# kshedden/muscato

Measured on AMD Instinct MI355X. Metric: reads/sec (100 bp, multi-map) at 1/2/4/8 MI355X; confirm-kernel HBM GB/s vs peak, higher is better.
Workload: dtype u32

## Files before the change

include/muscato_hip.h:

```cpp
#ifndef MUSCATO_HIP_H
#define MUSCATO_HIP_H

#include <stdint.h>

#ifdef __cplusplus
extern "C" {
#endif

#define MUSC_ABI_VERSION 3
#define MUSC_MAX_WINDOWS 16

typedef struct musc_ctx musc_ctx;

typedef struct {
  uint32_t read_idx;
  uint32_t gene_idx;
  uint32_t pos;
  uint32_t nmiss;
} musc_hit;

typedef struct {
  int32_t n_windows;
  int32_t windows[MUSC_MAX_WINDOWS];
  int32_t window_width;
// ... 53 lines not shown
int musc_db_build_index_for(musc_ctx* ctx, const musc_params* params, int32_t max_read_len);

int musc_db_set_partition_bases(musc_ctx* ctx, uint64_t max_bases);
int musc_db_partitions(musc_ctx* ctx, uint32_t* first_target, uint32_t cap, uint32_t* n);

int musc_reads_load_ascii(musc_ctx* ctx, const char* seqs, const uint64_t* offsets,
                          uint64_t nreads, int on_device);
int musc_reads_load_packed(musc_ctx* ctx, const uint8_t* bases2bit, const uint8_t* nmask,
                           const uint64_t* read_offsets, uint64_t nreads);
int musc_reads_load_packed32(musc_ctx* ctx, const uint8_t* bases2bit, const uint8_t* nmask,
                             const uint32_t* lengths, uint32_t fixed_len, uint64_t nreads, int async);

int musc_reads_sort_unique(musc_ctx* ctx, const char* seqs, const uint64_t* offsets, uint64_t nreads,
                           int on_device, uint32_t** order, uint32_t** ustart, uint64_t* nunique);

typedef struct musc_fastq_prep {
  uint64_t n_records, n_short, n_reads, n_unique;
  uint32_t max_len, reserved;
  uint64_t *name_off, *seq_off;
  uint32_t *name_len, *seq_len;
  uint32_t *order, *ustart;
} musc_fastq_prep;
int  musc_reads_prep_fastq(musc_ctx* ctx, const char* text, uint64_t nbytes, int on_device,
                           int32_t min_read_len, int32_t max_read_len, musc_fastq_prep* out);
void musc_fastq_prep_free(musc_fastq_prep* p);

int musc_reads_names_order(musc_ctx* ctx, const char* text, uint64_t nbytes, int on_device, const uint64_t* name_off,
                           const uint32_t* name_len, uint64_t n, const uint32_t* order, const uint32_t* ustart, uint64_t nu,
                           uint32_t* ranked_out);
typedef struct musc_read_names {
// ... 103 lines not shown
```

muscato_amd/_lib.py:

```python
from __future__ import annotations

import ctypes
import os

HERE = os.path.dirname(os.path.abspath(__file__))
LIB_PATH = os.environ.get("MUSC_LIB_PATH") or os.path.join(HERE, "libmuscato_hip.so")

MUSC_MAX_WINDOWS = 16


class MuscHit(ctypes.Structure):
    _fields_ = [("read_idx", ctypes.c_uint32), ("gene_idx", ctypes.c_uint32),
                ("pos", ctypes.c_uint32), ("nmiss", ctypes.c_uint32)]


class MuscParams(ctypes.Structure):
    _fields_ = [
        ("n_windows", ctypes.c_int32),
        ("windows", ctypes.c_int32 * MUSC_MAX_WINDOWS),
        ("window_width", ctypes.c_int32),
        ("pmatch", ctypes.c_double),
        ("min_dinuc", ctypes.c_int32),
        ("max_read_length", ctypes.c_int32),
        ("max_matches", ctypes.c_int32),
# ... 55 lines not shown

class MuscTargetsPrepInfo(ctypes.Structure):
    _fields_ = [
        ("n_lines", ctypes.c_uint64), ("n_records", ctypes.c_uint64), ("n_targets", ctypes.c_uint64),
        ("n_dropped", ctypes.c_uint64), ("stop_line", ctypes.c_uint64), ("n_subx", ctypes.c_uint64),
        ("n_seq_bytes", ctypes.c_uint64), ("n_id_bytes", ctypes.c_uint64),
        ("ms", ctypes.c_float), ("reserved", ctypes.c_uint32),
    ]


SYMBOLS = [
    "musc_abi_version", "musc_init", "musc_destroy", "musc_last_error", "musc_reload_env",
    "musc_db_load_ascii", "musc_db_load_packed", "musc_db_build_index", "musc_db_build_index_for",
    "musc_db_set_partition_bases", "musc_db_partitions",
    "musc_reads_load_ascii", "musc_reads_load_packed", "musc_reads_load_packed32", "musc_reads_sort_unique",
    "musc_reads_prep_fastq", "musc_fastq_prep_free",
    "musc_reads_names_order", "musc_reads_prep_fastq_names", "musc_reads_names_text",
    "musc_match_device", "musc_hits_copy", "musc_hits_copy_packed", "musc_hits_copy_compact", "musc_hits_unpack", "musc_match", "musc_free_hits",
    "musc_get_stats", "musc_last_instance", "musc_instances", "musc_stream_plan", "musc_gather", "musc_gather_rccl", "musc_rccl_probe", "musc_overflow_probes", "musc_free_u32",
    "musc_results_set_gene_text", "musc_results_set_read_text", "musc_results_order", "musc_results_hits", "musc_results_text",
    "musc_results_last_ms", "musc_results_number_key",
    "musc_side_prepare", "musc_side_text", "musc_side_last_ms",
    "musc_maxmatches_apply", "musc_maxmatches_last_ms", "musc_maxmatches_last_detail",
    "musc_sz_decode", "musc_db_load_text",
    "musc_targets_prep", "musc_targets_prep_text", "musc_targets_prep_load", "musc_targets_prep_free", "musc_sz_frame",
]

SIDE_NONMATCH, SIDE_GENESTATS, SIDE_READSTATS = 0, 1, 2

_lib = None

# ... 25 lines not shown
    lib.musc_destroy.restype = None
    lib.musc_last_error.argtypes = [vp]
    lib.musc_last_error.restype = ctypes.c_char_p
    lib.musc_reload_env.argtypes = [vp]
    lib.musc_db_load_ascii.argtypes = [vp, vp, vp, ctypes.c_uint32, ctypes.c_int]
    lib.musc_db_load_packed.argtypes = [vp, vp, vp, vp, ctypes.c_uint32]
    lib.musc_db_build_index.argtypes = [vp, i32]
    lib.musc_db_build_index_for.argtypes = [vp, ctypes.POINTER(MuscParams), i32]
    lib.musc_db_set_partition_bases.argtypes = [vp, u64]
    lib.musc_db_partitions.argtypes = [vp, vp, ctypes.c_uint32, ctypes.POINTER(ctypes.c_uint32)]
    lib.musc_reads_load_ascii.argtypes = [vp, vp, vp, u64, ctypes.c_int]
    lib.musc_reads_load_packed.argtypes = [vp, vp, vp, vp, u64]
    lib.musc_reads_load_packed32.argtypes = [vp, vp, vp, vp, ctypes.c_uint32, u64, ctypes.c_int]
    lib.musc_reads_sort_unique.argtypes = [vp, vp, vp, u64, ctypes.c_int, ctypes.POINTER(vp), ctypes.POINTER(vp),
                                           ctypes.POINTER(u64)]
    lib.musc_reads_prep_fastq.argtypes = [vp, vp, u64, ctypes.c_int, i32, i32, ctypes.POINTER(MuscFastqPrep)]
    lib.musc_reads_prep_fastq.restype = ctypes.c_int
    lib.musc_fastq_prep_free.argtypes = [ctypes.POINTER(MuscFastqPrep)]
    lib.musc_fastq_prep_free.restype = None
    lib.musc_reads_names_order.argtypes = [vp, vp, u64, ctypes.c_int, vp, vp, u64, vp, vp, u64, vp]
    lib.musc_reads_prep_fastq_names.argtypes = [vp, vp, u64, ctypes.c_int, i32, i32, ctypes.POINTER(MuscFastqPrep), ctypes.POINTER(MuscReadNames)]
    lib.musc_reads_names_text.argtypes = [vp, ctypes.c_int, u64, u64, vp, u64, ctypes.c_int, ctypes.POINTER(u64)]
    for name in ("musc_reads_names_order", "musc_reads_prep_fastq_names", "musc_reads_names_text"):
        getattr(lib, name).restype = ctypes.c_int
    lib.musc_match_device.argtypes = [vp, ctypes.POINTER(MuscParams), ctypes.POINTER(u64)]
    lib.musc_hits_copy.argtypes = [vp, vp, u64, ctypes.c_int]
    lib.musc_hits_copy_packed.argtypes = [vp, vp, u64, ctypes.c_int, u64, ctypes.POINTER(i32)]
    lib.musc_hits_copy_compact.argtypes = [vp, vp, u64, vp, u64, ctypes.c_int, ctypes.POINTER(i32)]
    lib.musc_hits_unpack.argtypes = [vp, vp, u64, ctypes.c_int, ctypes.POINTER(i32), vp]
    lib.musc_match.argtypes = [vp, ctypes.POINTER(MuscParams), ctypes.POINTER(vp), ctypes.POINTER(u64)]
# ... 54 lines not shown
```

muscato_amd/api.py:

```python
from __future__ import annotations

import ctypes
import json
from dataclasses import dataclass, field, asdict
from typing import List, Optional, Sequence, Tuple

import numpy as np

from . import _lib


class MuscatoError(RuntimeError):
    pass


@dataclass
class DbTextInfo:
    n_targets: int
    n_bases: int
    n_odd: int
    first_odd_target: int
    n_text_bytes: int
    n_chunks: int
    ms_decode: float
# ... 302 lines not shown

    def sort_unique_reads_arrays(self, seqs_ptr: int, off_ptr: int, nreads: int, on_device: bool):
        po, pu, nu = ctypes.c_void_p(), ctypes.c_void_p(), ctypes.c_uint64()
        self._check(self._lib.musc_reads_sort_unique(self._h, seqs_ptr, off_ptr, nreads, 1 if on_device else 0,
                                                     ctypes.byref(po), ctypes.byref(pu), ctypes.byref(nu)),
                    "musc_reads_sort_unique")
        try:
            order = np.ctypeslib.as_array(ctypes.cast(po, ctypes.POINTER(ctypes.c_uint32)), shape=(max(nreads, 1),))[:nreads].copy()
            ustart = np.ctypeslib.as_array(ctypes.cast(pu, ctypes.POINTER(ctypes.c_uint32)), shape=(nu.value + 1,)).copy()
        finally:
            self._lib.musc_free_u32(po)
            self._lib.musc_free_u32(pu)
        self.n_reads = int(nu.value)
        return order, ustart

    def prep_fastq(self, raw: bytes, min_len: int, max_len: int) -> dict:
        buf = np.frombuffer(raw, dtype=np.uint8)
        return self.prep_fastq_device(buf.ctypes.data if len(buf) else None, len(buf), min_len, max_len, on_device=False)

    def prep_fastq_device(self, ptr: Optional[int], nbytes: int, min_len: int, max_len: int, on_device: bool = True) -> dict:
        fp = _lib.MuscFastqPrep()
        self.n_reads = 0
        self._check(self._lib.musc_reads_prep_fastq(self._h, ptr, int(nbytes), 1 if on_device else 0, int(min_len), int(max_len),
                                                    ctypes.byref(fp)), "musc_reads_prep_fastq")
        try:
            n, nu = int(fp.n_reads), int(fp.n_unique)

            def arr(p, count):
                return np.ctypeslib.as_array(p, shape=(max(count, 1),))[:count].copy()
            out = {"n_records": int(fp.n_records), "n_short": int(fp.n_short), "n_reads": n, "n_unique": nu,
# ... 308 lines not shown
```

muscato_amd/build.py:

```python
from __future__ import annotations

import os
import shutil
import subprocess
from concurrent.futures import ThreadPoolExecutor

HERE = os.path.dirname(os.path.abspath(__file__))
CSRC = os.path.join(HERE, "csrc")
LIB = os.path.join(HERE, "libmuscato_hip.so")
OBJ = os.path.join(HERE, "build")
SOURCES = [os.path.join(CSRC, f) for f in ("muscato_hip.hip", "match_lane_rw4.hip", "match_lane_rw8.hip", "match_lane_rw12.hip",
                                           "match_lane_rw8w.hip", "match_lane_rw12w.hip", "match_lane_rw16w.hip", "match_lane_rw8s.hip", "match_dma_rw8.hip")]
HEADERS = [os.path.join(os.path.dirname(HERE), "include", "muscato_hip.h")] + \
    [os.path.join(CSRC, f) for f in sorted(os.listdir(CSRC)) if f.endswith(".hpp")]
LANE_ONLY = os.path.join(CSRC, "kernels_match_lane.hpp")
DMA_ONLY = os.path.join(CSRC, "kernels_match_dma.hpp")
FLAGS = ["--offload-arch=gfx950", "-O3", "-std=c++17", "-fPIC", "-Wall", "-Wno-unused-function"]


def hipcc() -> str:
    for cand in (shutil.which("hipcc"), "/opt/rocm/bin/hipcc"):
        if cand and os.path.exists(cand):
            return cand
    raise RuntimeError("hipcc not found: libmuscato_hip.so cannot be built")
# ... 27 lines not shown
            cmd += ["-L" + HERE, "-lmuscato_hip", "-Wl,-rpath,$ORIGIN/.."]
        if verbose:
            print(" ".join(cmd))
        subprocess.check_call(cmd)


_API = "../../include/muscato_hip.h"
_HOST_CHAIN = ("host/muscato_host.hpp", "host/cli_config.hpp", "host/cli_maxmatches_host.hpp", "host/cli_names.hpp", "host/cli_plan.hpp",
               "host/cli_text.hpp", "host/sz.hpp", _API)
CHECKS = {
    "cli_plan_check": ("cli_plan_check.cpp", ("host/check.hpp", "host/cli_names.hpp", "host/cli_plan.hpp"), 184_205_945, ()),
    "ctx_state_check": ("ctx_state_check.cpp", ("host/check.hpp", "ctx_state.hpp", _API), 58_376_821, ()),
    "dev_mem_check": ("dev_mem_check.cpp", ("host/check.hpp", "dev_mem.hpp"), 521, ()),
    "index_plan_check": ("index_plan_check.cpp", ("host/check.hpp", "index_plan.hpp"), 567_030, ()),
    "launch_plan_check": ("launch_plan_check.cpp", ("host/check.hpp", "launch_plan.hpp"), 113_302_959, ()),
    "load_plan_check": ("load_plan_check.cpp", ("host/check.hpp", "load_plan.hpp"), 35_240_767, ()),
    "maxmatches_plan_check": ("maxmatches_plan_check.cpp", ("host/check.hpp", "maxmatches_plan.hpp"), 548_365, ()),
    "read_names_plan_check": ("read_names_plan_check.cpp", ("host/check.hpp", "read_names_keys.hpp", "read_names_lanes.hpp", "read_names_plan.hpp"), 21_928_502, ()),
    "side_names_check": ("side_names_check.cpp", ("host/check.hpp", "side_names.hpp"), 100_517, ()),
    "sz_plan_check": ("sz_plan_check.cpp", ("host/check.hpp", "sz_plan.hpp", "host/sz.hpp"), 3_599_466, ("-lz",)),
    "targets_prep_plan_check": ("targets_prep_plan_check.cpp", ("host/check.hpp", "sz_plan.hpp", "targets_prep_plan.hpp") + _HOST_CHAIN, 12_757_977, ("-lz",)),
    "text_stage_check": ("text_stage_check.cpp", ("host/check.hpp", "text_stage.hpp"), 1_711_086, ()),
}
SANITIZE = ["-O1", "-g", "-fsanitize=address,undefined", "-fno-sanitize-recover=all", "-static-libasan", "-static-libubsan"]


def check_headers(name: str) -> list:
    return [os.path.normpath(os.path.join(CSRC, h)) for h in CHECKS[name][1]]


def build_checks(force: bool = False, verbose: bool = False, sanitize: bool = False, out_dir: str = BIN) -> dict:
# ... 66 lines not shown
```

muscato_amd/csrc/host/load_plan_check.cpp:

```cpp
#include <cstdio>
#include <cstdlib>
#include <vector>

#include "../load_plan.hpp"
#include "check.hpp"

namespace {

namespace ml = musc_load;


void check_shape(uint64_t maxlen) {
  ml::RecShape s;
  EXPECT(ml::rec_shape(1000, maxlen, &s) == ml::SHAPE_OK);
  EXPECT(s.rw % 4 == 0 && s.rw >= 4);
  EXPECT((uint64_t)(s.rw - 1) * 32 >= 2 * maxlen);
  EXPECT(s.rw == 4 || (uint64_t)(s.rw - 4 - 1) * 32 < 2 * maxlen);
  EXPECT(s.words == 1000ull * (uint64_t)s.rw);
}

void check_refusals() {
  ml::RecShape s;
  EXPECT(ml::rec_shape(0xFFFFFFF0ull, 0, &s) == ml::TOO_MANY_READS);
  EXPECT(ml::rec_shape(0xFFFFFFF0ull, 70000, &s) == ml::TOO_MANY_READS);
  EXPECT(ml::rec_shape(0xFFFFFFEFull, 0, &s) == ml::TOO_MANY_WORDS);
  EXPECT(ml::rec_shape(1, 65535, &s) == ml::SHAPE_OK && s.rw == 4100);
  EXPECT(ml::rec_shape(1, 65536, &s) == ml::READ_TOO_LONG);
  EXPECT(ml::rec_shape(0, 65536, &s) == ml::READ_TOO_LONG);
  EXPECT(ml::rec_shape((1ull << 30) - 1, 10, &s) == ml::SHAPE_OK && s.words == (1ull << 32) - 4);
  EXPECT(ml::rec_shape(1ull << 30, 10, &s) == ml::TOO_MANY_WORDS);
  EXPECT(ml::rec_shape((1ull << 29) - 1, 100, &s) == ml::SHAPE_OK && s.rw == 8);
  EXPECT(ml::rec_shape(1ull << 29, 100, &s) == ml::TOO_MANY_WORDS);
  EXPECT(ml::rec_shape(0, 0, &s) == ml::SHAPE_OK && s.rw == 4 && s.words == 0);
}


void check_db(uint64_t nbases) {
  const uint64_t w = ml::db_words(nbases);
  EXPECT(w * 16 >= nbases && (w == 0 || (w - 1) * 16 < nbases));
  EXPECT(ml::db_plane_words(w) == w + 64);
  const uint64_t blocks = ml::dbx_blocks(w);
  EXPECT(blocks * 4 >= ml::db_plane_words(w) && (blocks - 1) * 4 < ml::db_plane_words(w));
  EXPECT(ml::dbx_words(w) > (blocks - 1) / 32 + 1);
}


void check_stream(uint64_t nreads, uint32_t L, uint64_t batch_reads) {
  ml::StreamPlan sp;
// ... 45 lines not shown
  lens.push_back(65535);
  std::vector<uint64_t> counts = {0, 1, 2, 63};
  for (uint64_t m = 64; m <= 4096; m += 64)
    for (uint64_t d : {m - 1, m, m + 1}) counts.push_back(d);
  for (uint32_t L : lens) {
    check_shape(L);
    for (uint64_t n : counts)
      for (uint64_t batch : {1ull, 64ull, 100ull, 1000ull, 4096ull, 16ull << 20}) check_stream(n, L, batch);
    ml::RecShape s;
    EXPECT(ml::rec_shape(1, L, &s) == ml::SHAPE_OK);
    const uint64_t most = ((1ull << 32) - 1) / (uint64_t)s.rw;
    EXPECT(ml::rec_shape(most, L, &s) == ml::SHAPE_OK && ml::rec_shape(most + 1, L, &s) != ml::SHAPE_OK);
    for (uint64_t n : {most - 1, most, (uint64_t)0xFFFFFFEFull}) check_stream(n, L, 16ull << 20);
  }
  check_shape(0);
  for (uint64_t nb = 0; nb <= 5000; nb++) check_db(nb);
  for (uint64_t nb : {(1ull << 32) - 1, 1ull << 32, (1ull << 36) - 1}) check_db(nb);
  return check_done("load_plan_check");
}
```

muscato_amd/csrc/load_plan.hpp:

```cpp
#pragma once

#include <algorithm>
#include <cstdint>
#include <vector>

namespace musc_load {

enum Refusal { SHAPE_OK = 0, TOO_MANY_READS, READ_TOO_LONG, TOO_MANY_WORDS };
struct RecShape { int rw = 4; uint64_t words = 0; };
inline Refusal rec_shape(uint64_t nreads, uint64_t maxlen, RecShape* s) {
  if (nreads >= 0xFFFFFFF0ull) return TOO_MANY_READS;
  if (maxlen > 65535) return READ_TOO_LONG;
  s->rw = std::max(((int)((2 * maxlen + 31) / 32) + 1 + 3) & ~3, 4);
  s->words = nreads * (uint64_t)s->rw;
  if (s->words >= (1ull << 32)) return TOO_MANY_WORDS;
  return SHAPE_OK;
}

constexpr uint64_t DB_SLACK_WORDS = 64;
inline uint64_t db_words(uint64_t nbases) { return (nbases + 15) / 16; }
inline uint64_t db_plane_words(uint64_t words) { return words + DB_SLACK_WORDS; }
inline uint64_t dbx_blocks(uint64_t words) { return (db_plane_words(words) + 3) / 4; }
inline uint64_t dbx_words(uint64_t words) { return dbx_blocks(words) / 32 + 4; }

struct StreamPlan {
  std::vector<uint64_t> piece_end, batch_end;
};
inline void stream_plan(uint64_t nreads, uint64_t batch_reads, StreamPlan* sp) {
  auto up64 = [](uint64_t x) { return (x + 63) & ~63ull; };
  sp->piece_end.clear();
  sp->batch_end.clear();
// ... 26 lines not shown
```

muscato_amd/csrc/muscato_hip.hip:

```cpp

#include <hip/hip_runtime.h>
#include <rocprim/device/device_radix_sort.hpp>
#include <rccl/rccl.h>
#include <dlfcn.h>

#include <algorithm>
#include <cstdarg>
#include <cstdio>
#include <cstdlib>
#include <cstring>
#include <map>
#include <memory>
#include <mutex>
#include <string>
#include <type_traits>
#include <vector>

#include "../../include/muscato_hip.h"

#include "ctx_state.hpp"
#include "dev_mem.hpp"
#include "index_plan.hpp"
#include "launch_plan.hpp"
#include "load_plan.hpp"
// ... 89 lines not shown
  bool match_dma = false;
  bool screen_wg = false;
  int context = 0;
  bool no_x_context = false;
  bool force_wide = false;
  int debug_grid = 0;
  bool debug_sync = false;
  int graph = -1;
  bool pipeline = false;
  bool no_spec = false;
  long batch_reads = 0;
  uint64_t stage_bytes = 64ull << 20;
  uint64_t stage_lines = 1ull << 20;
  long mm_heap_lds = 0;
  uint64_t stage_grid = 0;
  void read() {
    *this = EnvKnobs();
    auto is = [](const char* v, const char* w) { return v && !strcmp(v, w); };
    const char* e = getenv("MUSC_INDEX");
    index = is(e, "classic") ? musc_index::IDX_CLASSIC : is(e, "lines") ? musc_index::IDX_LINES : is(e, "classic64") ? musc_index::IDX_CLASSIC64 : musc_index::IDX_AUTO;
    e = getenv("MUSC_MATCH");
    match_dma = is(e, "dma");
    screen_wg = is(getenv("MUSC_SCREEN"), "wg");
    e = getenv("MUSC_CONTEXT");
    context = is(e, "narrow") ? 1 : is(e, "wide") ? 2 : 0;
    no_x_context = getenv("MUSC_NO_X_CONTEXT") != nullptr;
    force_wide = getenv("MUSC_DEBUG_FORCE_WIDE") != nullptr;
    if ((e = getenv("MUSC_DEBUG_INDEX_BITS"))) index_bits = atoi(e);
    ctx_direct = (e = getenv("MUSC_DEBUG_CTX_DIRECT")) && atoi(e) > 0;
    if ((e = getenv("MUSC_DEBUG_GRID"))) debug_grid = atoi(e);
    debug_sync = getenv("MUSC_DEBUG_SYNC") != nullptr;
    if ((e = getenv("MUSC_GRAPH"))) graph = atoi(e);
    if ((e = getenv("MUSC_PIPELINE"))) pipeline = atoi(e) > 0;
    no_spec = getenv("MUSC_NO_SPEC") != nullptr;
    if ((e = getenv("MUSC_BATCH_READS"))) batch_reads = atol(e);
    if ((e = getenv("MUSC_DEBUG_INDEX_BUDGET_MB"))) index_budget_mb = atol(e);
    if ((e = getenv("MUSC_DEBUG_STAGE_BYTES")) && atoll(e) > 0) stage_bytes = (uint64_t)atoll(e);
    if ((e = getenv("MUSC_DEBUG_STAGE_LINES")) && atoll(e) > 0) stage_lines = (uint64_t)atoll(e);
    if ((e = getenv("MUSC_DEBUG_MM_HEAP_LDS"))) mm_heap_lds = atol(e);
    if ((e = getenv("MUSC_DEBUG_STAGE_GRID")) && atoll(e) > 0) stage_grid = std::min<uint64_t>((uint64_t)atoll(e), musc_launch::KNOB_MAX);
  }
};

struct musc_ctx {
  int device = 0;
  hipStream_t stream = nullptr;
  std::string err;
  EnvKnobs env;
  musc_state::State st;

  DevPtr<uint32_t> db2;
  DevPtr<uint32_t> dbm2;
  bool db_has_x = false;
  bool reads_have_x = false;
  DevBuf<uint32_t> rdx;
// ... 29 lines not shown
  PathParams h_pp;
  bool h_pp_valid = false;
  DevPtr<MatchParams> d_mp;
  MatchParams h_mp;
  bool h_mp_valid = false;
  int spec_geom = 0;
  DevBuf<uint4> spill;

  DevPtr<uint32_t> rd;
  uint64_t rd_cap = 0;
  DevPtr<uint32_t> rdm;
  uint64_t nreads = 0;
  int rw = 0;
  uint32_t max_len = 0;
  bool reads_failed = false;

  struct Upload {
    DevPtr<uint32_t> stage;
    hipStream_t s_up = nullptr;
    std::vector<hipEvent_t> ev;
    StreamPlan plan;
    uint64_t next_piece = 0;
    uint64_t packed_upto = 0;
    uint32_t L = 0;
    bool active = false;
  } up;

  struct BatchSet {
    DevBuf<uint32_t> wb, rvalid, tbase, tcount;
    DevBuf<uint4> cdesc;
// ... 151 lines not shown
int scan_u32(musc_ctx* c, const uint32_t* in, uint32_t* out, uint64_t n, bool inclusive, uint32_t* tmp, hipStream_t st = nullptr) {
  return scan_levels<uint32_t>(c, in, out, n, tmp, st ? st : c->stream, inclusive ? k_scan_block<true> : k_scan_block<false>, k_scan_block<false>, k_scan_add);
}

int scan_u64(musc_ctx* c, const uint64_t* in, uint64_t* out, uint64_t n, uint64_t* tmp) {
  return scan_levels<uint64_t>(c, in, out, n, tmp, c->stream, k_scan64_block, k_scan64_block, k_scan64_add);
}

template <class T>
int tmp_alloc(musc_ctx* c, const char* who, TmpBufs& B, T** ptr, uint64_t bytes) {
  const hipError_t e = B.alloc(ptr, bytes);
  if (e == hipSuccess) return 0;
  (void)hipGetLastError();
  return fail(c, 10, "%s: device allocation of %llu bytes failed: %s", who, (unsigned long long)bytes, hipGetErrorString(e));
}

template <class T>
int staged(musc_ctx* c, const char* who, TmpBufs& B, const T* ptr, uint64_t bytes, int on_device, uint64_t slack, const T** d_ptr) {
  *d_ptr = ptr;
  if (on_device) return 0;
  T* d = nullptr;
  const int rc = tmp_alloc(c, who, B, &d, bytes + slack);
  if (rc) return rc;
  if (bytes) HIPCHK(c, hipMemcpyAsync(d, ptr, bytes, hipMemcpyHostToDevice, c->stream));
  *d_ptr = d;
  return 0;
}

struct KeyPasses {
  TmpBufs B;
// ... 63 lines not shown
void drop_reads(musc_ctx* c, bool keep_rd) {
  if (c->up.active) {
    (void)hipStreamSynchronize(c->up.s_up);
    c->up.active = false;
  }
  if (!(keep_rd && c->rd_cap)) {
    c->rd.release();
    c->rd_cap = 0;
  }
  c->rdm.release();
  drop_read_text(c);
  c->reads_have_x = false;
  c->reads_failed = false;
  c->nreads = 0;
  c->rw = 0;
  c->st.reads_dropped();
}
void free_reads(musc_ctx* c) { drop_reads(c, false); }

int reads_load_done(musc_ctx* c, int rc) {
  if (rc) {
    if (c->up.s_up) (void)hipStreamSynchronize(c->up.s_up);
    (void)hipStreamSynchronize(c->stream);
    free_reads(c);
    c->reads_failed = true;
  }
  return rc;
}

struct EvPair {
// ... 793 lines not shown
```

muscato_amd/csrc/muscato_prep.hpp:

```cpp

#define PREP_BASES_PER_WORD 21

DEV uint32_t prep_code(unsigned char ch) {
  switch (ch) {
    case 'A': return 1u;
    case 'C': return 2u;
    case 'G': return 3u;
    case 'T': return 4u;
    default: return 5u;
  }
}

MUSC_KERNEL __launch_bounds__(256) void k_prep_keys(const unsigned char* __restrict__ s,
                                                   const uint64_t* __restrict__ off,
                                                   const uint32_t* __restrict__ perm, uint64_t n, uint32_t w,
                                                   uint64_t* __restrict__ keys) {
  for (uint64_t i = (uint64_t)blockIdx.x * blockDim.x + threadIdx.x; i < n; i += (uint64_t)gridDim.x * blockDim.x) {
    const uint32_t r = perm[i];
    const uint64_t o = off[r];
    const uint64_t len = off[r + 1] - o;
    const uint64_t first = (uint64_t)w * PREP_BASES_PER_WORD;
    uint64_t key = 0;
    for (uint32_t j = 0; j < PREP_BASES_PER_WORD; j++) {
      const uint64_t q = first + j;
      if (q >= len) break;
      key |= (uint64_t)prep_code(s[o + q]) << (60 - 3 * j);
    }
    keys[i] = key;
  }
}

MUSC_KERNEL __launch_bounds__(256) void k_prep_heads(const unsigned char* __restrict__ s,
                                                    const uint64_t* __restrict__ off,
                                                    const uint32_t* __restrict__ perm, uint64_t n,
                                                    uint32_t* __restrict__ head) {
  for (uint64_t i = (uint64_t)blockIdx.x * blockDim.x + threadIdx.x; i < n; i += (uint64_t)gridDim.x * blockDim.x) {
    uint32_t h = 1;
    if (i > 0) {
      const uint32_t a = perm[i], b = perm[i - 1];
      const uint64_t oa = off[a], ob = off[b];
      const uint64_t la = off[a + 1] - oa, lb = off[b + 1] - ob;
      if (la == lb) {
        h = 0;
// ... 54 lines not shown
  rd[t] = v;
  rdm[t] = mv;
  if (mv) atomicOr(has_x, 1u);
}

static int reads_sort_unique_dev(musc_ctx* c, const char* who, const unsigned char* d_s, const uint64_t* d_off, const uint64_t n,
                                 const Marks& m, uint32_t** order, uint32_t** ustart, uint64_t* nunique) {
  TmpBufs B;
  RecShape shape;
  uint64_t first = 0, last = 0, maxlen = 0;
  int rc = offsets_census(c, d_off, n, &first, &last, &maxlen);
  if (rc) return rc;
  if (first != 0) return fail(c, 2, "read offsets[0] must be 0");
  if ((rc = reads_shape(c, 0, maxlen, false, &shape))) return rc;

  const uint32_t nw = (uint32_t)std::max<uint64_t>((maxlen + PREP_BASES_PER_WORD - 1) / PREP_BASES_PER_WORD, 1);
  KeyPasses K;
  if ((rc = K.start(c, who, n, {63u}))) return rc;
  for (uint32_t w = nw; w-- > 0 && !rc;)
    rc = K.pass(63u, [&](const uint32_t* perm, uint64_t* keys) { hipLaunchKernelGGL(k_prep_keys, grid(c, n), dim3(256), 0, c->stream, d_s, d_off, perm, n, w, keys); });
  if (rc) return rc;
  const uint32_t* const p0 = K.order();

  uint32_t *head = nullptr, *incl = nullptr, *stmp = nullptr, *d_ustart = nullptr, *d_uhead = nullptr;
  if ((rc = tmp_alloc(c, who, B, &head, n * 4)) || (rc = tmp_alloc(c, who, B, &incl, n * 4)) ||
      (rc = tmp_alloc(c, who, B, &stmp, scan_tmp_elems(n) * 4)) || (rc = tmp_alloc(c, who, B, &d_ustart, (n + 1) * 4)) ||
      (rc = tmp_alloc(c, who, B, &d_uhead, n * 4)))
    return rc;
  hipLaunchKernelGGL(k_prep_heads, grid(c, n), dim3(256), 0, c->stream, d_s, d_off, p0, n, head);
  HIPCHK(c, hipGetLastError());
  if ((rc = scan_u32(c, head, incl, n, true, stmp))) return rc;
  hipLaunchKernelGGL(k_prep_starts, grid(c, n), dim3(256), 0, c->stream, head, incl, n, d_ustart, d_uhead, p0);
  HIPCHK(c, hipGetLastError());
  uint64_t nu = 0;
  HIPCHK(c, Readback(c->scalars, c->stream).get(incl + (n - 1), &nu).wait());

  if ((rc = reads_shape(c, nu, maxlen, false, &shape)) || (rc = reads_records(c, shape, nu, maxlen, true, false))) return rc;
  const auto [rw, words] = shape;
  uint32_t* d_hasx = c->d_flag;
  HIPCHK(c, hipMemsetAsync(d_hasx, 0, 4, c->stream));
  hipLaunchKernelGGL(k_prep_pack, dim3(nblk(words, 256)), dim3(256), 0, c->stream, d_s, d_off, d_uhead, nu, rw, c->rd,
                     c->rdm, d_hasx);
  HIPCHK(c, hipGetLastError());
  HIPCHK(c, m.mark(c, 1));

  std::unique_ptr<uint32_t, decltype(&free)> h_order((uint32_t*)malloc(n * 4), free), h_ustart((uint32_t*)malloc((nu + 1) * 4), free);
  if (!h_order || !h_ustart) return fail(c, 7, "out of host memory for the sort order");
  uint32_t hasx = 0;
  hipError_t e = hipMemcpyAsync(h_order.get(), p0, n * 4, hipMemcpyDeviceToHost, c->stream);
  if (e == hipSuccess) e = hipMemcpyAsync(h_ustart.get(), d_ustart, (nu + 1) * 4, hipMemcpyDeviceToHost, c->stream);
  const hipError_t ew = Readback(c->scalars, c->stream).get(d_hasx, &hasx).wait();
  if (e == hipSuccess) e = ew;
  if (e != hipSuccess) return fail(c, 10, "musc_reads_sort_unique: %s", hipGetErrorString(e));
  reads_settle_x(c, hasx);
  c->stats.ms_read_prep = m.ms(0, 1);
  *order = h_order.release();
  *ustart = h_ustart.release();
  *nunique = nu;
  return 0;
}

static int reads_sort_unique_run(musc_ctx* c, const char* seqs, const uint64_t* offsets, uint64_t nreads, int on_device,
                                 uint32_t** order, uint32_t** ustart, uint64_t* nunique) {
  HIPCHK(c, hipSetDevice(c->device));
  free_reads(c);
  if (nreads >= 0xFFFFFFF0ull) return fail(c, 2, "too many reads for 32-bit read numbers");
  if (nreads == 0) {
    c->rw = 4;
    *order = (uint32_t*)malloc(4);
// ... 11 lines not shown
  if ((rc = staged(c, who, B, (const unsigned char*)seqs, on_device ? 0 : offsets[nreads], on_device, 64, &d_s)) ||
      (rc = staged(c, who, B, offsets, (nreads + 1) * 8, on_device, 0, &d_off)))
    return rc;
  HIPCHK(c, m.mark(c, 0));
  return reads_sort_unique_dev(c, who, d_s, d_off, nreads, m, order, ustart, nunique);
}

extern "C" int musc_reads_sort_unique(musc_ctx* c, const char* seqs, const uint64_t* offsets, uint64_t nreads,
                                      int on_device, uint32_t** order, uint32_t** ustart, uint64_t* nunique) {
  if (!c) return 1;
  if (!order || !ustart || !nunique) return fail(c, 2, "musc_reads_sort_unique: NULL output pointer");
  *order = *ustart = nullptr;
  *nunique = 0;
  if ((!seqs || !offsets) && nreads) return fail(c, 2, "musc_reads_sort_unique: NULL input");
  return reads_load_done(c, reads_sort_unique_run(c, seqs, offsets, nreads, on_device, order, ustart, nunique));
}


extern "C" void musc_fastq_prep_free(musc_fastq_prep* p) {
  if (!p) return;
  free(p->name_off);
  free(p->seq_off);
  free(p->name_len);
  free(p->seq_len);
  free(p->order);
  free(p->ustart);
  memset(p, 0, sizeof *p);
}

template <class After>
// ... 92 lines not shown
```

Measured before the change: 2.102 billion.

## Pre-encode read keys once and reuse them across sort passes and head detection

Read sort/unique prep now encodes every read into packed 3-bit words in one coalesced pass using wide 8-byte loads. Each radix key pass then gathers from that buffer instead of re-reading and re-encoding the text, and duplicate-head detection compares the packed words. This removes repeated byte-wise text decoding per pass, at the cost of an n*nw*8-byte temporary buffer and a host readback of an odd-byte flag. When allocation fails or non-ACGTX bytes appear, it falls back to the old kernels.

```diff
diff --git a/include/muscato_hip.h b/include/muscato_hip.h
--- a/include/muscato_hip.h
+++ b/include/muscato_hip.h
@@ -91,6 +91,10 @@
 int musc_reads_sort_unique(musc_ctx* ctx, const char* seqs, const uint64_t* offsets, uint64_t nreads,
                            int on_device, uint32_t** order, uint32_t** ustart, uint64_t* nunique);
 
+#define MUSC_PREP_DETAIL_WORDS 4
+enum { MUSC_PREP_ENCODED = 0, MUSC_PREP_KNOB = 1, MUSC_PREP_NO_ROOM = 2, MUSC_PREP_ODD_BYTES = 3 };
+int musc_reads_prep_last_detail(const musc_ctx* ctx, uint32_t* out);
+
 typedef struct musc_fastq_prep {
   uint64_t n_records, n_short, n_reads, n_unique;
   uint32_t max_len, reserved;
diff --git a/muscato_amd/_lib.py b/muscato_amd/_lib.py
--- a/muscato_amd/_lib.py
+++ b/muscato_amd/_lib.py
@@ -93,7 +93,7 @@
     "musc_db_load_ascii", "musc_db_load_packed", "musc_db_build_index", "musc_db_build_index_for",
     "musc_db_set_partition_bases", "musc_db_partitions",
     "musc_reads_load_ascii", "musc_reads_load_packed", "musc_reads_load_packed32", "musc_reads_sort_unique",
-    "musc_reads_prep_fastq", "musc_fastq_prep_free",
+    "musc_reads_prep_last_detail", "musc_reads_prep_fastq", "musc_fastq_prep_free",
     "musc_reads_names_order", "musc_reads_prep_fastq_names", "musc_reads_names_text",
     "musc_match_device", "musc_hits_copy", "musc_hits_copy_packed", "musc_hits_copy_compact", "musc_hits_unpack", "musc_match", "musc_free_hits",
     "musc_get_stats", "musc_last_instance", "musc_instances", "musc_stream_plan", "musc_gather", "musc_gather_rccl", "musc_rccl_probe", "musc_overflow_probes", "musc_free_u32",
@@ -149,6 +149,8 @@
     lib.musc_reads_load_packed32.argtypes = [vp, vp, vp, vp, ctypes.c_uint32, u64, ctypes.c_int]
     lib.musc_reads_sort_unique.argtypes = [vp, vp, vp, u64, ctypes.c_int, ctypes.POINTER(vp), ctypes.POINTER(vp),
                                            ctypes.POINTER(u64)]
+    lib.musc_reads_prep_last_detail.argtypes = [vp, ctypes.POINTER(ctypes.c_uint32)]
+    lib.musc_reads_prep_last_detail.restype = ctypes.c_int
     lib.musc_reads_prep_fastq.argtypes = [vp, vp, u64, ctypes.c_int, i32, i32, ctypes.POINTER(MuscFastqPrep)]
     lib.musc_reads_prep_fastq.restype = ctypes.c_int
     lib.musc_fastq_prep_free.argtypes = [ctypes.POINTER(MuscFastqPrep)]
diff --git a/muscato_amd/api.py b/muscato_amd/api.py
--- a/muscato_amd/api.py
+++ b/muscato_amd/api.py
@@ -340,6 +340,12 @@
         self.n_reads = int(nu.value)
         return order, ustart
 
+    def read_prep_detail(self) -> dict:
+        w = (ctypes.c_uint32 * 4)()
+        self._check(self._lib.musc_reads_prep_last_detail(self._h, w), "musc_reads_prep_last_detail")
+        return {"sort_encoded": bool(w[0]), "groups_encoded": bool(w[1]), "fallback": ("none", "knob", "no_room", "odd_bytes")[w[2]],
+                "has_x": bool(w[3])}
+
     def prep_fastq(self, raw: bytes, min_len: int, max_len: int) -> dict:
         buf = np.frombuffer(raw, dtype=np.uint8)
         return self.prep_fastq_device(buf.ctypes.data if len(buf) else None, len(buf), min_len, max_len, on_device=False)
diff --git a/muscato_amd/build.py b/muscato_amd/build.py
--- a/muscato_amd/build.py
+++ b/muscato_amd/build.py
@@ -65,7 +65,7 @@
     "dev_mem_check": ("dev_mem_check.cpp", ("host/check.hpp", "dev_mem.hpp"), 521, ()),
     "index_plan_check": ("index_plan_check.cpp", ("host/check.hpp", "index_plan.hpp"), 567_030, ()),
     "launch_plan_check": ("launch_plan_check.cpp", ("host/check.hpp", "launch_plan.hpp"), 113_302_959, ()),
-    "load_plan_check": ("load_plan_check.cpp", ("host/check.hpp", "load_plan.hpp"), 35_240_767, ()),
+    "load_plan_check": ("load_plan_check.cpp", ("host/check.hpp", "load_plan.hpp"), 35_406_059, ()),
     "maxmatches_plan_check": ("maxmatches_plan_check.cpp", ("host/check.hpp", "maxmatches_plan.hpp"), 548_365, ()),
     "read_names_plan_check": ("read_names_plan_check.cpp", ("host/check.hpp", "read_names_keys.hpp", "read_names_lanes.hpp", "read_names_plan.hpp"), 21_928_502, ()),
     "side_names_check": ("side_names_check.cpp", ("host/check.hpp", "side_names.hpp"), 100_517, ()),
diff --git a/muscato_amd/csrc/host/load_plan_check.cpp b/muscato_amd/csrc/host/load_plan_check.cpp
--- a/muscato_amd/csrc/host/load_plan_check.cpp
+++ b/muscato_amd/csrc/host/load_plan_check.cpp
@@ -32,6 +32,22 @@
   EXPECT(ml::rec_shape((1ull << 29) - 1, 100, &s) == ml::SHAPE_OK && s.rw == 8);
   EXPECT(ml::rec_shape(1ull << 29, 100, &s) == ml::TOO_MANY_WORDS);
   EXPECT(ml::rec_shape(0, 0, &s) == ml::SHAPE_OK && s.rw == 4 && s.words == 0);
+}
+
+
+void check_prep_words(uint64_t maxlen) {
+  const uint64_t nw = ml::prep_key_words(maxlen);
+  EXPECT(nw >= 1 && nw * ml::PREP_WORD_BASES >= maxlen);
+  EXPECT(nw == 1 || (nw - 1) * ml::PREP_WORD_BASES < maxlen);
+}
+
+void check_prep_encode(uint64_t n, uint64_t nw) {
+  uint64_t bytes = 77;
+  const unsigned __int128 words = (unsigned __int128)n * nw;
+  const bool fits = ml::prep_encode_bytes(n, nw, &bytes);
+  EXPECT(fits == (nw != 0 && words <= (unsigned __int128)(~0ull >> 3)));
+  EXPECT(bytes == (fits ? (uint64_t)words * 8 : 0));
+  if (fits && n) EXPECT(bytes / 8 / nw == n && bytes % 8 == 0 && (n - 1) * nw + (nw - 1) < bytes / 8);
 }
 
 
@@ -107,6 +123,21 @@
     for (uint64_t n : {most - 1, most, (uint64_t)0xFFFFFFEFull}) check_stream(n, L, 16ull << 20);
   }
   check_shape(0);
+  for (uint64_t L = 0; L <= 70000; L++) check_prep_words(L);
+  EXPECT(ml::prep_key_words(0) == 1 && ml::prep_key_words(21) == 1 && ml::prep_key_words(22) == 2 && ml::prep_key_words(100) == 5 &&
+         ml::prep_key_words(105) == 5 && ml::prep_key_words(65535) == 3121);
+  {
+    const std::vector<uint64_t> ns = {0, 1, 2, 255, 50000000, (1ull << 29) - 1, 1ull << 29, 0xFFFFFFEFull, 1ull << 32, (1ull << 61) - 1, 1ull << 61, ~0ull};
+    const std::vector<uint64_t> nws = {0, 1, 2, 5, 8, 3121, (1ull << 29) + 1, 1ull << 32, (1ull << 61) - 1, 1ull << 61, ~0ull};
+    for (uint64_t n : ns)
+      for (uint64_t nw : nws) check_prep_encode(n, nw);
+    for (uint64_t nw = 1; nw <= 3121; nw++)
+      for (uint64_t n : {(uint64_t)((~0ull >> 3) / nw), (uint64_t)((~0ull >> 3) / nw + 1), (uint64_t)0xFFFFFFEFull}) check_prep_encode(n, nw);
+    uint64_t b = 0;
+    EXPECT(ml::prep_encode_bytes(50000000, 5, &b) && b == 2000000000ull);
+    EXPECT(ml::prep_encode_bytes(0xFFFFFFEFull, 3121, &b) && b > (1ull << 46));
+    EXPECT(!ml::prep_encode_bytes(1ull << 40, 1ull << 21, &b) && b == 0);
+  }
   for (uint64_t nb = 0; nb <= 5000; nb++) check_db(nb);
   for (uint64_t nb : {(1ull << 32) - 1, 1ull << 32, (1ull << 36) - 1}) check_db(nb);
   return check_done("load_plan_check");
diff --git a/muscato_amd/csrc/load_plan.hpp b/muscato_amd/csrc/load_plan.hpp
--- a/muscato_amd/csrc/load_plan.hpp
+++ b/muscato_amd/csrc/load_plan.hpp
@@ -15,6 +15,15 @@
   s->words = nreads * (uint64_t)s->rw;
   if (s->words >= (1ull << 32)) return TOO_MANY_WORDS;
   return SHAPE_OK;
+}
+
+constexpr uint64_t PREP_WORD_BASES = 21;
+inline uint64_t prep_key_words(uint64_t maxlen) { return std::max<uint64_t>(maxlen / PREP_WORD_BASES + (maxlen % PREP_WORD_BASES != 0), 1); }
+inline bool prep_encode_bytes(uint64_t n, uint64_t nw, uint64_t* bytes) {
+  *bytes = 0;
+  if (nw == 0 || (n != 0 && nw > (~0ull >> 3) / n)) return false;
+  *bytes = n * nw * 8;
+  return true;
 }
 
 constexpr uint64_t DB_SLACK_WORDS = 64;
diff --git a/muscato_amd/csrc/muscato_hip.hip b/muscato_amd/csrc/muscato_hip.hip
--- a/muscato_amd/csrc/muscato_hip.hip
+++ b/muscato_amd/csrc/muscato_hip.hip
@@ -127,6 +127,7 @@
   uint64_t stage_lines = 1ull << 20;
   long mm_heap_lds = 0;
   uint64_t stage_grid = 0;
+  bool prep_encode = true;
   void read() {
     *this = EnvKnobs();
     auto is = [](const char* v, const char* w) { return v && !strcmp(v, w); };
@@ -152,6 +153,7 @@
     if ((e = getenv("MUSC_DEBUG_STAGE_LINES")) && atoll(e) > 0) stage_lines = (uint64_t)atoll(e);
     if ((e = getenv("MUSC_DEBUG_MM_HEAP_LDS"))) mm_heap_lds = atol(e);
     if ((e = getenv("MUSC_DEBUG_STAGE_GRID")) && atoll(e) > 0) stage_grid = std::min<uint64_t>((uint64_t)atoll(e), musc_launch::KNOB_MAX);
+    if ((e = getenv("MUSC_DEBUG_PREP_ENCODE"))) prep_encode = atoi(e) != 0;
   }
 };
 
@@ -211,6 +213,7 @@
   int rw = 0;
   uint32_t max_len = 0;
   bool reads_failed = false;
+  uint32_t prep_detail[MUSC_PREP_DETAIL_WORDS] = {0, 0, 0, 0};
 
   struct Upload {
     DevPtr<uint32_t> stage;
@@ -392,6 +395,10 @@
   (void)hipGetLastError();
   return fail(c, 10, "%s: device allocation of %llu bytes failed: %s", who, (unsigned long long)bytes, hipGetErrorString(e));
 }
+template <class T>
+void tmp_alloc_soft(TmpBufs& B, T** ptr, uint64_t bytes) {
+  if (B.alloc(ptr, bytes) != hipSuccess) (void)hipGetLastError(), *ptr = nullptr;
+}
 
 template <class T>
 int staged(musc_ctx* c, const char* who, TmpBufs& B, const T* ptr, uint64_t bytes, int on_device, uint64_t slack, const T** d_ptr) {
@@ -485,6 +492,7 @@
   c->reads_failed = false;
   c->nreads = 0;
   c->rw = 0;
+  memset(c->prep_detail, 0, sizeof c->prep_detail);
   c->st.reads_dropped();
 }
 void free_reads(musc_ctx* c) { drop_reads(c, false); }
diff --git a/muscato_amd/csrc/muscato_prep.hpp b/muscato_amd/csrc/muscato_prep.hpp
--- a/muscato_amd/csrc/muscato_prep.hpp
+++ b/muscato_amd/csrc/muscato_prep.hpp
@@ -2,13 +2,37 @@
 #define PREP_BASES_PER_WORD 21
 
 DEV uint32_t prep_code(unsigned char ch) {
-  switch (ch) {
-    case 'A': return 1u;
-    case 'C': return 2u;
-    case 'G': return 3u;
-    case 'T': return 4u;
-    default: return 5u;
-  }
+  uint32_t c = 5u;
+  c = ch == 'T' ? 4u : c;
+  c = ch == 'G' ? 3u : c;
+  c = ch == 'C' ? 2u : c;
+  c = ch == 'A' ? 1u : c;
+  return c;
+}
+
+DEV uint32_t prep_word_bases(uint64_t len, uint32_t w) {
+  const uint64_t first = (uint64_t)w * PREP_BASES_PER_WORD;
+  return first >= len ? 0u : (uint32_t)(len - first < PREP_BASES_PER_WORD ? len - first : PREP_BASES_PER_WORD);
+}
+
+template <bool PADDED, class ByteAt>
+DEV uint64_t prep_key_word(uint32_t cnt, ByteAt byte_at, uint32_t* odd) {
+  uint64_t key = 0;
+  uint32_t other = 0;
+#pragma unroll
+  for (uint32_t j = 0; j < PREP_BASES_PER_WORD; j++) {
+    if (!PADDED && j >= cnt) break;
+    const unsigned char ch = byte_at(j);
+    const uint32_t code = prep_code(ch);
+    other |= (uint32_t)(code == 5u && ch != 'X') << j;
+    key |= (uint64_t)code << (60 - 3 * j);
+  }
+  if (PADDED) {
+    key &= cnt ? ~0ull << (63 - 3 * cnt) : 0ull;
+    other &= (1u << cnt) - 1u;
+  }
+  *odd |= (uint32_t)(other != 0);
+  return key;
 }
 
 MUSC_KERNEL __launch_bounds__(256) void k_prep_keys(const unsigned char* __restrict__ s,
@@ -19,14 +43,62 @@
     const uint32_t r = perm[i];
     const uint64_t o = off[r];
     const uint64_t len = off[r + 1] - o;
-    const uint64_t first = (uint64_t)w * PREP_BASES_PER_WORD;
+    const unsigned char* const p = s + o + (uint64_t)w * PREP_BASES_PER_WORD;
+    uint32_t odd = 0;
+    keys[i] = prep_key_word<false>(prep_word_bases(len, w), [p](uint32_t j) { return p[j]; }, &odd);
+  }
+}
+
+MUSC_KERNEL __launch_bounds__(256) void k_prep_encode(const unsigned char* __restrict__ s, const uint64_t* __restrict__ off, uint64_t n,
+                                                     uint32_t nw, uint64_t total, uint64_t* __restrict__ enc,
+                                                     uint32_t* __restrict__ odd_flag) {
+  const uint64_t words = n * nw;
+  uint32_t odd = 0;
+  for (uint64_t base = (uint64_t)blockIdx.x * 256; base < words; base += (uint64_t)gridDim.x * 256) {
+    const uint32_t x = (uint32_t)(base % nw) + threadIdx.x;
+    const uint64_t r = base / nw + x / nw;
+    const uint32_t w = x % nw;
+    if (r >= n) continue;
+    const uint64_t o = off[r];
+    const uint32_t cnt = prep_word_bases(off[r + 1] - o, w);
+    const uint64_t a = o + (uint64_t)w * PREP_BASES_PER_WORD;
     uint64_t key = 0;
-    for (uint32_t j = 0; j < PREP_BASES_PER_WORD; j++) {
-      const uint64_t q = first + j;
-      if (q >= len) break;
-      key |= (uint64_t)prep_code(s[o + q]) << (60 - 3 * j);
-    }
-    keys[i] = key;
+    if (cnt && a + 24 <= total) {
+      uint64_t q0, q1, q2;
+      __builtin_memcpy(&q0, s + a, 8);
+      __builtin_memcpy(&q1, s + a + 8, 8);
+      __builtin_memcpy(&q2, s + a + 16, 8);
+      key = prep_key_word<true>(cnt, [=](uint32_t j) { return (unsigned char)((j < 8 ? q0 : j < 16 ? q1 : q2) >> (8 * (j & 7))); }, &odd);
+    } else if (cnt) {
+      const unsigned char* const p = s + a;
+      key = prep_key_word<false>(cnt, [p](uint32_t j) { return p[j]; }, &odd);
+    }
+    enc[r * nw + w] = key;
+  }
+  if (odd) atomicOr(odd_flag, 1u);
+}
+
+MUSC_KERNEL __launch_bounds__(256) void k_prep_fill(const uint64_t* __restrict__ enc, const uint32_t* __restrict__ perm, uint64_t n,
+                                                   uint32_t nw, uint32_t w, uint64_t* __restrict__ keys) {
+  for (uint64_t i = (uint64_t)blockIdx.x * blockDim.x + threadIdx.x; i < n; i += (uint64_t)gridDim.x * blockDim.x)
+    keys[i] = enc[(uint64_t)perm[i] * nw + w];
+}
+
+MUSC_KERNEL __launch_bounds__(256) void k_prep_heads_enc(const uint64_t* __restrict__ enc, const uint32_t* __restrict__ perm,
+                                                        uint64_t n, uint32_t nw, uint32_t* __restrict__ head) {
+  for (uint64_t i = (uint64_t)blockIdx.x * blockDim.x + threadIdx.x; i < n; i += (uint64_t)gridDim.x * blockDim.x) {
+    uint32_t h = 1;
+    if (i > 0) {
+      const uint64_t* const a = enc + (uint64_t)perm[i] * nw;
+      const uint64_t* const b = enc + (uint64_t)perm[i - 1] * nw;
+      h = 0;
+      for (uint32_t w = 0; w < nw; w++)
+        if (a[w] != b[w]) {
+          h = 1;
+          break;
+        }
+    }
+    head[i] = h;
   }
 }
 
@@ -111,11 +183,31 @@
   if (first != 0) return fail(c, 2, "read offsets[0] must be 0");
   if ((rc = reads_shape(c, 0, maxlen, false, &shape))) return rc;
 
-  const uint32_t nw = (uint32_t)std::max<uint64_t>((maxlen + PREP_BASES_PER_WORD - 1) / PREP_BASES_PER_WORD, 1);
+  const uint32_t nw = (uint32_t)musc_load::prep_key_words(maxlen);
+  uint32_t why = c->env.prep_encode ? MUSC_PREP_ENCODED : MUSC_PREP_KNOB;
+  uint64_t* enc = nullptr;
+  uint32_t* d_odd = nullptr;
+  uint64_t enc_bytes = 0;
+  if (c->env.prep_encode) {
+    if (musc_load::prep_encode_bytes(n, nw, &enc_bytes)) tmp_alloc_soft(B, &enc, enc_bytes);
+    if (!enc) why = MUSC_PREP_NO_ROOM;
+  }
+  if (enc) {
+    if ((rc = tmp_alloc(c, who, B, &d_odd, 4))) return rc;
+    HIPCHK(c, hipMemsetAsync(d_odd, 0, 4, c->stream));
+    hipLaunchKernelGGL(k_prep_encode, grid(c, n * nw), dim3(256), 0, c->stream, d_s, d_off, n, nw, last, enc, d_odd);
+    HIPCHK(c, hipGetLastError());
+  }
+
   KeyPasses K;
   if ((rc = K.start(c, who, n, {63u}))) return rc;
   for (uint32_t w = nw; w-- > 0 && !rc;)
-    rc = K.pass(63u, [&](const uint32_t* perm, uint64_t* keys) { hipLaunchKernelGGL(k_prep_keys, grid(c, n), dim3(256), 0, c->stream, d_s, d_off, perm, n, w, keys); });
+    rc = K.pass(63u, [&](const uint32_t* perm, uint64_t* keys) {
+      if (enc)
+        hipLaunchKernelGGL(k_prep_fill, grid(c, n), dim3(256), 0, c->stream, (const uint64_t*)enc, perm, n, nw, w, keys);
+      else
+        hipLaunchKernelGGL(k_prep_keys, grid(c, n), dim3(256), 0, c->stream, d_s, d_off, perm, n, w, keys);
+    });
   if (rc) return rc;
   const uint32_t* const p0 = K.order();
 
@@ -124,7 +216,14 @@
       (rc = tmp_alloc(c, who, B, &stmp, scan_tmp_elems(n) * 4)) || (rc = tmp_alloc(c, who, B, &d_ustart, (n + 1) * 4)) ||
       (rc = tmp_alloc(c, who, B, &d_uhead, n * 4)))
     return rc;
-  hipLaunchKernelGGL(k_prep_heads, grid(c, n), dim3(256), 0, c->stream, d_s, d_off, p0, n, head);
+  uint32_t odd = 0;
+  if (enc) HIPCHK(c, Readback(c->scalars, c->stream).get(d_odd, &odd).wait());
+  if (odd) why = MUSC_PREP_ODD_BYTES;
+  const bool by_words = enc && !odd;
+  if (by_words)
+    hipLaunchKernelGGL(k_prep_heads_enc, grid(c, n), dim3(256), 0, c->stream, (const uint64_t*)enc, p0, n, nw, head);
+  else
+    hipLaunchKernelGGL(k_prep_heads, grid(c, n), dim3(256), 0, c->stream, d_s, d_off, p0, n, head);
   HIPCHK(c, hipGetLastError());
   if ((rc = scan_u32(c, head, incl, n, true, stmp))) return rc;
   hipLaunchKernelGGL(k_prep_starts, grid(c, n), dim3(256), 0, c->stream, head, incl, n, d_ustart, d_uhead, p0);
@@ -150,6 +249,8 @@
   if (e == hipSuccess) e = ew;
   if (e != hipSuccess) return fail(c, 10, "musc_reads_sort_unique: %s", hipGetErrorString(e));
   reads_settle_x(c, hasx);
+  const uint32_t detail[MUSC_PREP_DETAIL_WORDS] = {enc != nullptr, by_words, why, hasx != 0};
+  memcpy(c->prep_detail, detail, sizeof detail);
   c->stats.ms_read_prep = m.ms(0, 1);
   *order = h_order.release();
   *ustart = h_ustart.release();
@@ -191,6 +292,12 @@
   *nunique = 0;
   if ((!seqs || !offsets) && nreads) return fail(c, 2, "musc_reads_sort_unique: NULL input");
   return reads_load_done(c, reads_sort_unique_run(c, seqs, offsets, nreads, on_device, order, ustart, nunique));
+}
+
+extern "C" int musc_reads_prep_last_detail(const musc_ctx* c, uint32_t* out) {
+  if (!c || !out) return 1;
+  memcpy(out, c->prep_detail, sizeof c->prep_detail);
+  return 0;
 }
 
 
diff --git a/profiles/read_prep.py b/profiles/read_prep.py
--- /dev/null
+++ b/profiles/read_prep.py
@@ -0,0 +1,92 @@
+#!/usr/bin/env python3
+import csv
+import json
+import os
+import statistics
+import sys
+
+ROOT = os.path.dirname(os.path.dirname(os.path.abspath(__file__)))
+sys.path.insert(0, ROOT)
+COPY_CEILING_TBPS = 6.29
+STAGE = ("k_prep_", "k_offsets_census", "k_scan_block", "k_scan_add", "rocprim", "radix", "onesweep")
+
+
+def run(workload, reps):
+    import torch
+    from muscato_amd import Engine, synth
+    wl = synth.workload_for(workload, 1)
+    device = torch.device("cuda", 0)
+    torch.cuda.set_device(0)
+    seed = synth.SEED_BASE + sum(ord(c) for c in wl.seed_key)
+    targets = synth.gen_targets(wl, device, seed)
+    U = wl.n_unique_reads
+    reads = synth.sort_reads(synth.gen_unique_reads(wl, targets, device, seed + 7919))
+    del targets
+    g = torch.Generator(device=device)
+    g.manual_seed(seed + 17)
+    n_raw = wl.n_raw_reads
+    extra = torch.randint(0, U, (n_raw - U,), device=device, generator=g)
+    raw = torch.cat([reads, reads[extra]])[torch.randperm(n_raw, device=device, generator=g)]
+    del extra, reads
+    raw_off = synth.offsets_for(n_raw, wl.read_len, device)
+    torch.cuda.synchronize()
+    torch.cuda.empty_cache()
+    ms = []
+    with Engine(0) as eng:
+        for _ in range(reps + 1):
+            order, ustart = eng.sort_unique_reads_arrays(raw.data_ptr(), raw_off.data_ptr(), n_raw, True)
+            ms.append(eng.stats()["ms_read_prep"])
+    return {"workload": workload, "raw_reads": n_raw, "read_len": wl.read_len, "text_bytes": int(raw.numel()),
+            "distinct": int(len(ustart) - 1), "calls": reps + 1, "device_ms": ms[1:], "device_ms_median": statistics.median(ms[1:])}
+
+
+def short(name):
+    for k in ("radix_sort_onesweep_iteration", "radix_sort_onesweep_global_offsets", "radix_sort_block_sort", "radix_sort_single"):
+        if k in name:
+            return "rocprim::" + k
+    return name.split("(")[0]
+
+
+def table(src, dst, calls):
+    rows, seen = [], {}
+    with open(src) as f:
+        for row in csv.DictReader(f):
+            if any(k in row["Name"] for k in STAGE) and "at::" not in row["Name"]:
+                name = short(row["Name"])
+                seen[name] = seen.get(name, 0) + 1
+                row["Name"] = name if seen[name] == 1 else "%s [%d]" % (name, seen[name])
+                rows.append(row)
+    total = sum(float(r["TotalDurationNs"]) for r in rows)
+    with open(dst, "w", newline="") as f:
+        w = csv.writer(f)
+        w.writerow(["Name", "Calls", "TotalDurationNs", "AverageNs", "MinNs", "MaxNs", "PercentOfStageKernels", "MsPerStageCall"])
+        for r in sorted(rows, key=lambda r: -float(r["TotalDurationNs"])):
+            t = float(r["TotalDurationNs"])
+            w.writerow([r["Name"], r["Calls"], r["TotalDurationNs"], r["AverageNs"], r["MinNs"], r["MaxNs"], "%.2f" % (100 * t / total),
+                        "%.3f" % (t / 1e6 / calls) if calls else ""])
+    return {"kernels": len(rows), "stage_kernel_ms": total / 1e6, "stage_kernel_ms_per_call": total / 1e6 / calls if calls else None}
+
+
+def rate(src, kernel, nbytes):
+    with open(src) as f:
+        for row in csv.DictReader(f):
+            if kernel in row["Name"]:
+                avg_ns = float(row["AverageNs"])
+                return {"kernel": kernel, "calls": int(row["Calls"]), "avg_us": avg_ns / 1e3, "bytes": nbytes, "TBps": nbytes / avg_ns / 1e3,
+                        "copy_ceiling_TBps": COPY_CEILING_TBPS}
+    raise SystemExit("no kernel %r in %s" % (kernel, src))
+
+
+def main():
+    a = sys.argv[1:]
+    if a and a[0] == "--table":
+        print(json.dumps(table(a[1], a[2], int(a[3]) if len(a) > 3 else 0)))
+    elif a and a[0] == "--rate":
+        print(json.dumps(rate(a[1], a[2], int(a[3]))))
+    else:
+        print(json.dumps(run(a[0] if a else "cfg3", int(a[1]) if len(a) > 1 else 3)), flush=True)
+    return 0
+
+
+if __name__ == "__main__":
+    sys.exit(main())
diff --git a/profiles/read_prep_ab.py b/profiles/read_prep_ab.py
--- /dev/null
+++ b/profiles/read_prep_ab.py
@@ -0,0 +1,87 @@
+#!/usr/bin/env python3
+import argparse
+import hashlib
+import json
+import os
+import statistics
+import subprocess
+import sys
+import tempfile
+import time
+
+ROOT = os.path.dirname(os.path.dirname(os.path.abspath(__file__)))
+
+
+def bench(where, extra, timeout):
+    env = {k: v for k, v in os.environ.items() if k != "PYTHONPATH"}
+    t0 = time.time()
+    r = subprocess.run([sys.executable, "bench.py", "--gpus", "1", "--steps", "20", "--warmup", "5"] + extra, cwd=where, env=env,
+                       stdout=subprocess.PIPE, stderr=subprocess.PIPE, timeout=timeout)
+    if r.returncode:
+        sys.stderr.write(r.stderr.decode()[-4000:])
+        raise SystemExit("bench.py in %s ended with %d: nothing more is started" % (where, r.returncode))
+    res = json.loads(r.stdout.decode().strip().splitlines()[-1])
+    one = res["one_off"]
+    rec = {"read_prep_device_ms": one["read_prep_device_ms"], "read_prep_wall_s": one["read_prep_wall_s"], "value": res["value"],
+           "distinct": one["distinct"], "wall_s": round(time.time() - t0, 1)}
+    if "--full" in extra:
+        rec.update(equals_torch_sort=one["equals_torch_sort"], ms_per_pass=res["kernel_pipeline"]["ms_per_pass"])
+    return rec
+
+
+def hashes(d):
+    out = {}
+    for f in sorted(os.listdir(d)):
+        with open(os.path.join(d, f), "rb") as fh:
+            out[f] = hashlib.sha1(fh.read()).hexdigest()
+    return out
+
+
+def main():
+    ap = argparse.ArgumentParser()
+    ap.add_argument("--parent", required=True)
+    ap.add_argument("--runs", type=int, default=5)
+    ap.add_argument("--out", default=os.path.join(ROOT, "profiles", "read_prep_encode_ab.jsonl"))
+    ap.add_argument("--timeout", type=int, default=300)
+    a = ap.parse_args()
+    builds = (("parent", os.path.abspath(a.parent)), ("this", ROOT))
+    recs = []
+    with open(a.out, "w") as out:
+        def put(rec):
+            recs.append(rec)
+            out.write(json.dumps(rec) + "\n")
+            out.flush()
+            print(json.dumps(rec), flush=True)
+
+        for i in range(a.runs):
+            for name, where in builds:
+                put(dict(bench(where, [], a.timeout), build=name, run=i, full=False))
+        with tempfile.TemporaryDirectory() as tmp:
+            for name, where in builds:
+                d = os.path.join(tmp, name)
+                put(dict(bench(where, ["--full", "--no-cpu-baseline", "--dump-outputs", d], 2 * a.timeout), build=name, run=0, full=True, dumped=hashes(d)))
+
+        def of(name, key, full=False):
+            return [r[key] for r in recs if r["build"] == name and r["full"] == full]
+
+        s = {"summary": True, "runs": a.runs}
+        for key in ("read_prep_device_ms", "read_prep_wall_s", "value"):
+            for name, _ in builds:
+                v = of(name, key)
+                s["%s_%s" % (key, name)] = {"median": statistics.median(v), "spread": max(v) - min(v), "min": min(v), "max": max(v)}
+        p, t = s["read_prep_device_ms_parent"], s["read_prep_device_ms_this"]
+        s["read_prep_device_ms_gain"] = p["median"] - t["median"]
+        s["gain_exceeds_three_spreads"] = abs(p["median"] - t["median"]) > 3 * max(p["spread"], t["spread"])
+        pv, tv = s["value_parent"], s["value_this"]
+        s["value_within_parent_spread"] = abs(tv["median"] - pv["median"]) <= pv["spread"]
+        fp, ft = [r for r in recs if r["full"] and r["build"] == "parent"][0], [r for r in recs if r["full"] and r["build"] == "this"][0]
+        s["ms_per_pass"] = {"parent": fp["ms_per_pass"], "this": ft["ms_per_pass"]}
+        s["equals_torch_sort"] = {"parent": fp["equals_torch_sort"], "this": ft["equals_torch_sort"]}
+        s["dumps_identical"] = fp["dumped"] == ft["dumped"] and len(fp["dumped"]) > 0
+        s["distinct_equal"] = len({r["distinct"] for r in recs}) == 1
+        put(s)
+    return 0
+
+
+if __name__ == "__main__":
+    sys.exit(main())
```

New measurement: 2.096 billion. Within noise of the previous version (-0.3%).
